# xu-ji/IIC

Measured on AMD Instinct MI355X. Metric: paired-images/sec, STL10 96x96 ClusterNet5g+IID_loss, higher is better.
Workload: dtype bf16; 1 GPU; STL10 96x96 ClusterNet5g IID+ (cluster_sobel.py train step), batch 660 pairs/GPU, 5 sub-heads, k=70, bf16 MFMA convs / fp32 stem+heads+loss, fused HIP Adam; global_batch_pairs=660, input=96x96x1 grey -> sobel 2ch, parallelism=dp1, streams=2, launch=hip-graph replay: 6 linear graph segments, the two views on two streams

## Files before the change

iic_amd/csrc/conv_igemm_bd.hip:

```cpp
#include "common.h"
#include "conv_plan.h"
#include "conv_tile.h"
#include "../../include/iic_hip.h"

template <int OFF>
__device__ __forceinline__ void bd_bload_at(u32x4& d, unsigned voff, const unsigned char* sbase) {
  asm volatile("global_load_dwordx4 %0, %1, %2 offset:%3" : "=v"(d) : "v"(voff), "s"(sbase), "n"(OFF) : "memory");
}
__device__ __forceinline__ void bd_bload(u32x4& d, unsigned voff, const unsigned char* sbase, int ks) {
  switch (ks) {
    case 0: bd_bload_at<0>(d, voff, sbase); break;
    case 1: bd_bload_at<1024>(d, voff, sbase); break;
    case 2: bd_bload_at<2048>(d, voff, sbase); break;
    default: bd_bload_at<3072>(d, voff, sbase); break;
  }
}
template <int N>
__device__ __forceinline__ void bd_bwait(u32x4& d) {
  asm volatile("s_waitcnt vmcnt(%1)" : "+v"(d) : "i"(N) : "memory");
}


#define BD_BM 256
#define BD_BN 128
// ... 326 lines not shown
  if (PROF) t_stamp[4] = __builtin_readcyclecounter();
  TileRed tr;
  if (RED) tile_red_zero(tr);
  if (!(ABL & 32))
    igemm_store_tile<BNT, BM, BD_THREADS, 8, RED, (BM == 256 ? BD_STORE_UB : 4)>(sC, s_pout, out, res_grad, res_act, accumulate,
                                                                 g.Cout, n0, tid, red_y, red_coef, red_y2, &tr);
  if (RED)
    igemm_red_finish<BNT, BD_THREADS, RED>(tr, reinterpret_cast<float*>(smem_raw), red_stats, red_stats2,
                                             g.Cout, n0, tid);
  if (PROF && prof && tid == 0) {
    unsigned long long* q = prof + (long)blockIdx.x * BD_PROF_SLOTS;
    const unsigned long long t_end = __builtin_readcyclecounter();
    q[0] = t_stamp[0]; q[1] = t_stamp[1]; q[2] = t_stamp[2]; q[3] = t_stamp[3]; q[4] = t_stamp[4];
    q[5] = t_end; q[6] = t_bsum; q[7] = (unsigned long long)t_nb;
    q[8] = iic_hw_stamp();
    q[9] = (unsigned long long)tix;
    q[10] = __builtin_amdgcn_s_memrealtime();
  }
}

template <bool GATHER, int ABL, int MS, int RED, int WN = 2, bool PAD = false>
__global__ __launch_bounds__(BD_THREADS, ((MS == 4 || WN == 1) ? 2 : 3)) void conv_igemm_bd_kernel(
    const iic_conv_geom g, const bf16_t* __restrict__ in, const unsigned char* __restrict__ wfrag,
    bf16_t* __restrict__ out, float* __restrict__ stats, const bf16_t* __restrict__ res_grad,
    const bf16_t* __restrict__ res_act, int accumulate, int num_mtiles, int lds_a_bytes,
    const bf16_t* __restrict__ red_y, const float* __restrict__ red_coef,
    const bf16_t* __restrict__ red_y2, float* __restrict__ red_stats, float* __restrict__ red_stats2,
    unsigned long long* __restrict__ prof, const bd_blk B) {
  bd_tile<GATHER, ABL, MS, RED, WN, PAD>(g, in, wfrag, out, stats, res_grad, res_act, accumulate, lds_a_bytes, red_y,
                                    red_coef, red_y2, red_stats, red_stats2, prof, (int)blockIdx.x,
                                    num_mtiles * (g.Cout / (WN * 64)), B);
}

__global__ void weight_prep_frag_kernel(const float* __restrict__ w, bf16_t* __restrict__ o, int Co,
                                        int Ci, int T, int mode) {
  const int Nn = mode ? Ci : Co, Kk = mode ? Co : Ci;
  const int n32 = Nn >> 5, nchunks = Kk >> 6;
  const long total = (long)T * Co * Ci;
  for (long i = (long)blockIdx.x * blockDim.x + threadIdx.x; i < total;
       i += (long)gridDim.x * blockDim.x) {
    const int e = (int)(i & 7), lane = (int)((i >> 3) & 63), ks = (int)((i >> 9) & 3);
    long r = i >> 11;
    const int j = (int)(r % n32);
    r /= n32;
    const int kc = (int)(r % nchunks), t = (int)(r / nchunks);
    const int n = j * 32 + (lane & 31), k = kc * 64 + ks * 16 + (lane >> 5) * 8 + e;
    const int co = mode ? k : n, ci = mode ? n : k;
    o[i] = f32_to_bf16(w[((long)co * Ci + ci) * T + t]);
  }
}

IIC_SWITCH(g_p64_enabled, 1, iic_debug_enable_p64)
IIC_SWITCH(g_p64_red, 0, iic_debug_p64_red)

extern "C" {

#ifdef IIC_DEBUG_HOOKS
static unsigned long long* g_bd_prof = nullptr;
IIC_HOOK void iic_debug_bd_prof(void* buf) { g_bd_prof = (unsigned long long*)buf; }
IIC_HOOK int iic_debug_bd_prof_slots(void) { return BD_PROF_SLOTS; }
#else
static constexpr unsigned long long* g_bd_prof = nullptr;
#endif

static long bd_lds(long npix, int rows, int couts, bool pad, bool keys, int* lds_a = nullptr) {
  const long a = pad ? pt144_bytes(npix) : (npix * 128 + 1023) & ~1023L;
  const long c = (long)rows * (couts + 8) * 2;
  const long la = ((a > c ? a : c) + 15) & ~15L;
  if (lds_a) *lds_a = (int)la;
  return la + 2L * rows * 4 + 4L * BD_BN * 4 + (keys ? (npix + 15) & ~15L : 0);
}
static long bd_lds_rows(const iic_conv_geom* g, int ms, int wn = 2, bool pad = false, int* lds_a = nullptr) {
  const int rows = ms * 32 * (4 / wn);
  const long npix = g->ntaps == 1 ? rows : (rows >= 192 ? g->NP256 : g->NP);
  const bool skip = g->ntaps > 1 && g->sx == 1 && ((g->in_Wp - g->MX) & 1) == 0 && g->in_Wp != g->MX;
  return bd_lds(npix, rows, wn * 64, pad, !pad && skip, lds_a);
}
IIC_SWITCH(g_bd_pitch144, IIC_BD_PITCH144, iic_debug_bd_pitch144)
#ifdef IIC_DEBUG_HOOKS
IIC_HOOK int iic_debug_get_bd_pitch144(void) { return g_bd_pitch144; }
#endif
static bool bd_pad_ok(const iic_conv_geom* g, int ms) {
// ... 180 lines not shown
    case 128: BD_LAUNCH(false, 128); break;
#endif
    default: BD_LAUNCH(false, 0); break;
  }
  return rc ? rc : iic_launch_status();
}

#ifdef IIC_DEBUG_HOOKS
IIC_HOOK void iic_debug_conv_plan(const iic_conv_geom* g, int* out) {
  conv_plan p;
  conv_make_plan(g, &p);
  const int f[12] = {p.kernel, p.ms, p.wn, p.gather, p.pad, p.blk.bw, p.blk.bh, p.mtiles, p.grid, p.lds_a, (int)p.lds,
                     p.red_ok};
  for (int i = 0; i < 12; ++i) out[i] = f[i];
}
IIC_HOOK int iic_debug_bd_pitch144_used(const iic_conv_geom* g) {
  conv_plan p;
  if (!conv_make_plan(g, &p) || !p.pad) return 0;
  return p.kernel == CONV_PW ? 2 : 1;
}
#endif

__global__ __launch_bounds__(256) void weight_prep_multi_kernel(const iic_weight_prep_job* __restrict__ jobs,
                                                                int njobs) {
  int lo = 0, hi = njobs - 1;
  while (lo < hi) {
    const int mid = (lo + hi + 1) >> 1;
    if ((long long)blockIdx.x >= jobs[mid].first_block) lo = mid; else hi = mid - 1;
  }
  const iic_weight_prep_job j = jobs[lo];
  const float* __restrict__ w = j.w;
  bf16_t* __restrict__ o = reinterpret_cast<bf16_t*>(j.out);
  const int Co = j.Cout, Ci = j.Cin, T = j.T, mode = j.mode;
  const long total = (long)T * Co * Ci;
  const long nblk = (total + 2047) >> 11;
  const long b = (long)blockIdx.x - j.first_block;
  if (b >= nblk) return;
  for (long i = b * 256 + threadIdx.x; i < total; i += nblk * 256) {
    if (mode <= 1) {
      const int Nn = mode ? Ci : Co, Kk = mode ? Co : Ci;
      const int n32 = Nn >> 5, nchunks = Kk >> 6;
      const int e = (int)(i & 7), lane = (int)((i >> 3) & 63), ks = (int)((i >> 9) & 3);
      long r = i >> 11;
      const int jj = (int)(r % n32);
      r /= n32;
      const int kc = (int)(r % nchunks), t = (int)(r / nchunks);
      const int n = jj * 32 + (lane & 31), k = kc * 64 + ks * 16 + (lane >> 5) * 8 + e;
      const int co = mode ? k : n, ci = mode ? n : k;
      o[i] = f32_to_bf16(w[((long)co * Ci + ci) * T + t]);
    } else if (mode == 2) {
      const int ci = (int)(i % Ci);
      const long r = i / Ci;
      const int co = (int)(r % Co), t = (int)(r / Co);
      o[i] = f32_to_bf16(w[((long)co * Ci + ci) * T + t]);
    } else {
      const int co = (int)(i % Co);
      const long r = i / Co;
      const int ci = (int)(r % Ci), t = (int)(r / Ci);
      o[i] = f32_to_bf16(w[((long)co * Ci + ci) * T + t]);
    }
  }
}

long iic_weight_prep_multi_blocks(int Cout, int Cin, int T) { return ((long)T * Cout * Cin + 2047) >> 11; }

int iic_weight_prep_multi(const iic_weight_prep_job* jobs_dev, int njobs, long total_blocks, void* stream) {
  if (!jobs_dev || njobs <= 0 || total_blocks <= 0 || total_blocks >= (1L << 31)) return IIC_ERR_ARG;
  hipLaunchKernelGGL(weight_prep_multi_kernel, dim3((unsigned)total_blocks), dim3(256), 0, (hipStream_t)stream,
                     jobs_dev, njobs);
  return iic_launch_status();
}

int iic_weight_prep_frag(const float* w_oihw, void* w_frag, int Cout, int Cin, int T, int bwd,
                         void* stream) {
  if (!w_oihw || !w_frag || Cout <= 0 || Cin <= 0 || T <= 0) return IIC_ERR_ARG;
  const int Nn = bwd ? Cin : Cout, Kk = bwd ? Cout : Cin;
  if (Nn % 32 != 0 || Kk % 64 != 0) return IIC_ERR_UNSUPPORTED;
  const long total = (long)T * Cout * Cin;
  int grid = (int)((total + 255) / 256);
  if (grid > 4096) grid = 4096;
  hipLaunchKernelGGL(weight_prep_frag_kernel, dim3(grid), dim3(256), 0, (hipStream_t)stream,
                     w_oihw, (bf16_t*)w_frag, Cout, Cin, T, bwd ? 1 : 0);
  return iic_launch_status();
}

}
```

iic_amd/csrc/conv_wgrad.hip:

```cpp
#include "common.h"
#include "conv_plan.h"
#include "conv_tile.h"
#include "../../include/iic_hip.h"

#define BM 128
#define TPG 3
#define NTG 3
#define PFX 4

typedef s16x4 __attribute__((address_space(3))) * lds_s16x4_ptr;

typedef uint16_t __attribute__((address_space(3))) * lds_u16_ptr;
template <bool USE_TR>
__device__ __forceinline__ bf16x8 frag_T(uint32_t a0, uint32_t a1, uint32_t tile, int pitch,
                                         const int* rows8, int col) {
  union { bf16x8 v; s16x4 h[2]; uint16_t e[8]; } u;
  if (USE_TR) {
    u.h[0] = __builtin_amdgcn_ds_read_tr16_b64_v4i16((lds_s16x4_ptr)(uintptr_t)a0);
    u.h[1] = __builtin_amdgcn_ds_read_tr16_b64_v4i16((lds_s16x4_ptr)(uintptr_t)a1);
  } else {
#pragma unroll
    for (int j = 0; j < 8; ++j)
      u.e[j] = *(lds_u16_ptr)(uintptr_t)(tile + rows8[j] * pitch + col * 2);
  }
  return u.v;
}

template <bool USE_TR, bool GATHER, int COT>
__global__ __launch_bounds__(GATHER ? 256 : 768) void conv_wgrad_kernel(
    const iic_conv_geom g, const bf16_t* __restrict__ x, const bf16_t* __restrict__ dy,
    float* __restrict__ partials, int nsplit, int num_ktiles, int lds_x_bytes) {
  constexpr int NT = GATHER ? 256 : 768;
  constexpr int CS = COT / 64;
  constexpr int DPITCH = COT == 64 ? 144 : 288;
  constexpr int DPIECES = BM * (COT / 8);
  constexpr int PDN = (DPIECES + NT - 1) / NT;
  constexpr int MYT = GATHER ? 1 : TPG;
  extern __shared__ __attribute__((aligned(16))) unsigned char smem_raw[];
  unsigned char* sX = smem_raw;
  unsigned char* sD = smem_raw + lds_x_bytes;
  int* s_pin = reinterpret_cast<int*>(sD + BM * DPITCH);
  int* s_pout = s_pin + 2 * BM;

  const int tid = threadIdx.x, lane = tid & 63, wave = tid >> 6;
  const int tg = wave >> 2, wm = (wave >> 1) & 1, wn = wave & 1;
  const int l31 = lane & 31, g5 = lane >> 5;
  const int q = lane >> 4, i16 = lane & 15;
  const int ncit = g.Cin >> 6;
  int tile = blockIdx.x, split = blockIdx.y;
  if ((gridDim.y & 7) == 0) {
    const int L = blockIdx.y * gridDim.x + blockIdx.x;
    const int xcd = L & 7, j = L >> 3;
    tile = j % (int)gridDim.x;
    split = xcd + 8 * (j / (int)gridDim.x);
  }
  const int cot = tile / ncit, cit = tile - cot * ncit;
  const int co0 = cot * COT, ci0 = cit * 64;
  const int per = (num_ktiles + nsplit - 1) / nsplit;
  const int kt0 = split * per;
  const int kt1 = min(num_ktiles, kt0 + per);
  const int in_pixels = g.N * g.in_Hp * g.in_Wp;
// ... 56 lines not shown
      }
    }
  };
  auto lstore_x = [&]() {
    const int tl = launder(tid);
#pragma unroll
    for (int u = 0; u < PFX; ++u) {
      const int idx = u * NT + tl;
      if (idx < n8) *reinterpret_cast<u32x4*>(sX + (idx >> 3) * ROWB + (idx & 7) * 16) = PX[u];
    }
  };
  auto load_x_sync_big = [&](int b) {
    const int p_lo = s_pin[b * BM];
    for (int base = 0; base < n8; base += NT * 4) {
      u32x4 v[4];
#pragma unroll
      for (int u = 0; u < 4; ++u) {
        const int idx = base + u * NT + tid;
        v[u] = (u32x4){0u, 0u, 0u, 0u};
        if (idx < n8) {
          const int p = p_lo + (idx >> 3);
          if (p < in_pixels)
            v[u] = *reinterpret_cast<const u32x4*>(x + ((long)p * g.Cin + ci0 + (idx & 7) * 8));
        }
      }
#pragma unroll
      for (int u = 0; u < 4; ++u) {
        const int idx = base + u * NT + tid;
        if (idx < n8) *reinterpret_cast<u32x4*>(sX + (idx >> 3) * ROWB + (idx & 7) * 16) = v[u];
      }
    }
  };

  for (int t0 = (int)blockIdx.z * (GATHER ? 1 : NTG * TPG), pass = 0; pass < 1; ++pass) {
    const int tfirst = t0 + tg * MYT;
    const int tcount = max(0, min(MYT, g.ntaps - tfirst));
    f32x16 acc[MYT][CS];
#pragma unroll
    for (int t = 0; t < MYT; ++t)
#pragma unroll
      for (int c = 0; c < CS; ++c)
#pragma unroll
        for (int r = 0; r < 16; ++r) acc[t][c][r] = 0.f;

    __syncthreads();
    if (kt0 < kt1) {
      rowinfo(kt0, 0);
      __syncthreads();
      gload_d(0);
      if (pf) { gload_x(0); lstore_x(); } else load_x_sync_big(0);
      lstore_d();
      if (kt0 + 1 < kt1) rowinfo(kt0 + 1, 1);
      __syncthreads();
    }
    for (int kt = kt0; kt < kt1; ++kt) {
      const int b = (kt - kt0) & 1;
      const bool more = kt + 1 < kt1;
      if (more) {
        gload_d(b ^ 1);
        if (pf) gload_x(b ^ 1);
      }
      const int p_lo = s_pin[b * BM];
      const int* spin = s_pin + b * BM;
#pragma unroll 2
      for (int ks = 0; ks < BM / 16; ++ks) {
        int rows8[8], rowsA[8];
// ... 72 lines not shown
    for (int u = 0; u < 8; ++u) a[u] = 0.f;
    int sp = 0;
    for (; sp + 8 <= nsplit; sp += 8) {
#pragma unroll
      for (int u = 0; u < 8; ++u) a[u] += partials[(long)(sp + u) * per + i];
    }
    for (; sp < nsplit; ++sp) a[0] += partials[(long)sp * per + i];
    const float s = ((a[0] + a[1]) + (a[2] + a[3])) + ((a[4] + a[5]) + (a[6] + a[7]));
    const int ci = (int)(i % Ci);
    const long r = i / Ci;
    const int co = (int)(r % Co), t = (int)(r / Co);
    const long o = ((long)co * Ci + ci) * T + t;
    dW[o] = accumulate ? dW[o] + s : s;
  }
}

__global__ void probe_tr16_kernel(uint16_t* out) {
  __shared__ __attribute__((aligned(16))) uint16_t lds[64 * 4];
  const int l = threadIdx.x;
  for (int i = l; i < 256; i += 64) lds[i] = (uint16_t)i;
  __syncthreads();
  const s16x4 v = __builtin_amdgcn_ds_read_tr16_b64_v4i16((lds_s16x4_ptr)(&lds[l * 4]));
  for (int j = 0; j < 4; ++j) out[l * 4 + j] = (uint16_t)v[j];
}

extern "C" {

#ifdef IIC_DEBUG_HOOKS
static int g_wgrad_target_wgs = 224;
IIC_HOOK void iic_debug_wgrad_target_wgs(int v) { g_wgrad_target_wgs = v > 0 ? v : 224; }
#else
static constexpr int g_wgrad_target_wgs = 224;
#endif

static int wgrad_reg_kt(const iic_conv_geom* g) { return (int)((igemm_rows_host(g) + BM - 1) / BM); }
static int wgrad_reg_batches(const iic_conv_geom* g) { return g->ntaps == 1 ? 1 : (g->ntaps + NTG * TPG - 1) / (NTG * TPG); }

int iic_conv_wgrad_nsplit(const iic_conv_geom* g) {
  const int kt = wgrad_reg_kt(g);
  const int tiles = (g->Cout / wgrad_cot(g)) * (g->Cin / 64) * wgrad_reg_batches(g);
  int ns = g_wgrad_target_wgs / (tiles > 0 ? tiles : 1);
  if (ns < 1) ns = 1;
  if (ns > kt) ns = kt;
  return ns;
}

static bool wgrad_make_plan(const iic_conv_geom* g, int use_tr, wgrad_plan* p) {
  *p = wgrad_plan{};
  if (!g || g->Cin % 64 != 0 || g->Cout % 64 != 0 || g->ntaps < 1 || g->ntaps > IIC_MAX_TAPS) return false;
  if (igemm_rows_host(g) >= (1L << 31) || (long)g->N * g->in_Hp * g->in_Wp >= (1L << 31)) return false;
  p->use_tr = use_tr != 0;
  p->cot = wgrad_cot(g);
  p->gx = (g->Cout / p->cot) * (g->Cin / 64);
  p->nsplit = iic_conv_wgrad_nsplit(g);
  if (use_tr && iic_wgrad_dma_plan(g, p)) return true;
  p->gather = g->ntaps == 1;
  p->bmk = BM; p->nbuf = 1;
  p->np = p->gather ? BM : g->NP;
  p->lx = (p->np * ROWB + 15) & ~15;
  p->lds = (long)p->lx + BM * (p->cot == 64 ? 144 : 288) + 4 * BM * 4;
  if (p->lds > IIC_LDS_BYTES) {
    *p = wgrad_plan{};
    return false;
  }
  p->kt = wgrad_reg_kt(g);
  p->gz = wgrad_reg_batches(g);
  p->threads = p->gather ? 256 : 768;
  p->kernel = WGRAD_REG;
  return true;
}

int iic_conv_wgrad(const iic_conv_geom* g, const void* x, const void* dy, float* partials,
                   int nsplit, int use_tr, void* stream) {
  if (!g || !x || !dy || !partials || nsplit < 1) return IIC_ERR_ARG;
  wgrad_plan p;
  if (!wgrad_make_plan(g, use_tr, &p)) return IIC_ERR_UNSUPPORTED;
  if (p.kernel != WGRAD_REG) return iic_wgrad_dma_launch(g, p, x, dy, partials, nsplit, stream);
  int rc = IIC_OK;
#define WGRAD_LAUNCH(TR_, GA_, COT_)                                                                           \
  rc = iic_launch_lds<conv_wgrad_kernel<TR_, GA_, COT_>>(dim3(p.gx, nsplit, p.gz), dim3(p.threads), p.lds,     \
                                                         (hipStream_t)stream, *g, (const bf16_t*)x,            \
                                                         (const bf16_t*)dy, partials, nsplit, p.kt, p.lx)
#define WGRAD_LAUNCH2(TR_, GA_)                                                                 \
  do {                                                                                          \
    if (p.cot == 128) WGRAD_LAUNCH(TR_, GA_, 128); else WGRAD_LAUNCH(TR_, GA_, 64);             \
  } while (0)
  if (p.use_tr) { if (p.gather) WGRAD_LAUNCH2(true, true); else WGRAD_LAUNCH2(true, false); }
  else          { if (p.gather) WGRAD_LAUNCH2(false, true); else WGRAD_LAUNCH2(false, false); }
  return rc ? rc : iic_launch_status();
}

#ifdef IIC_DEBUG_HOOKS
IIC_HOOK void iic_debug_wgrad_plan(const iic_conv_geom* g, int use_tr, int* out) {
  wgrad_plan p;
  wgrad_make_plan(g, use_tr, &p);
  const int f[28] = {p.kernel, p.band > 0, p.asm_reads, p.gather, p.cot, p.bmk, p.nbuf, p.ntab, p.txs, p.band,
                     p.bstride, p.mto, p.np, p.plane, p.lx, p.kt, p.gx, p.nsplit, p.gz, p.threads, (int)p.lds,
                     p.blk.bw, p.blk.bh, p.blk.nbx, p.blk.nby, p.blk.PW, p.blk.NPR, p.blk.drow};
  for (int i = 0; i < 28; ++i) out[i] = f[i];
}
#endif

int iic_conv_wgrad_reduce(const float* partials, int nsplit, int T, int Cout, int Cin, float* dW,
                          int accumulate, void* stream) {
  if (!partials || !dW || nsplit < 1) return IIC_ERR_ARG;
  const long per = (long)T * Cout * Cin;
  int grid = (int)((per + 255) / 256);
  if (grid > 4096) grid = 4096;
  hipLaunchKernelGGL(conv_wgrad_reduce_kernel, dim3(grid), dim3(256), 0, (hipStream_t)stream,
                     partials, nsplit, T, Cout, Cin, dW, accumulate);
  return iic_launch_status();
}

int iic_probe_tr16(void* out_u16_64x4, void* stream) {
  hipLaunchKernelGGL(probe_tr16_kernel, dim3(1), dim3(64), 0, (hipStream_t)stream,
                     (uint16_t*)out_u16_64x4);
  return iic_launch_status();
}

}
```

iic_amd/csrc/bn.hip:

```cpp
#include "common.h"
#include "../../include/iic_hip.h"

__device__ __forceinline__ void unpack8(const uint4 v, float* f) {
  f[0] = bf16lo(v.x); f[1] = bf16hi(v.x); f[2] = bf16lo(v.y); f[3] = bf16hi(v.y);
  f[4] = bf16lo(v.z); f[5] = bf16hi(v.z); f[6] = bf16lo(v.w); f[7] = bf16hi(v.w);
}
__device__ __forceinline__ uint4 pack8(const float* f) {
  return make_uint4(pack_bf16x2(f[0], f[1]), pack_bf16x2(f[2], f[3]), pack_bf16x2(f[4], f[5]),
                    pack_bf16x2(f[6], f[7]));
}

template <bool NT>
__device__ __forceinline__ uint4 ld16(const bf16_t* p) {
  if (NT) {
    const u32x4 v = __builtin_nontemporal_load(reinterpret_cast<const u32x4*>(p));
    return make_uint4(v[0], v[1], v[2], v[3]);
  }
  return *reinterpret_cast<const uint4*>(p);
}
__global__ __launch_bounds__(256) void bn_finalize_kernel(
    float* __restrict__ stats, const float* __restrict__ gamma, const float* __restrict__ beta,
    float* __restrict__ running_mean, float* __restrict__ running_var, long long* __restrict__ nbt,
    float* __restrict__ coef, int C, long count, long ucount, float eps, float momentum, int training) {
  const int lane16 = threadIdx.x & 15;
// ... 207 lines not shown
  unpack8(*reinterpret_cast<const uint4*>(y + off), v);
  if (act) {
    float a[8];
    unpack8(*reinterpret_cast<const uint4*>(act + off), a);
#pragma unroll
    for (int i = 0; i < 8; ++i) g[i] = a[i] > 0.f ? g[i] : 0.f;
  } else if (mcoef) {
    ld8(mcoef + c8 * 8, k1);
    ld8(mcoef + C + c8 * 8, k2);
#pragma unroll
    for (int i = 0; i < 8; ++i) g[i] = (v[i] * k1[i] + k2[i]) > 0.f ? g[i] : 0.f;
  }
  ld8(bcoef + c8 * 8, k1);
  ld8(bcoef + C + c8 * 8, k2);
  ld8(bcoef + 2 * C + c8 * 8, k3);
#pragma unroll
  for (int i = 0; i < 8; ++i) o[i] = k1[i] * g[i] + k2[i] * v[i] + k3[i];
  *reinterpret_cast<uint4*>(dy + off) = pack8(o);
  if (y2) {
    unpack8(*reinterpret_cast<const uint4*>(y2 + off), v);
    ld8(bcoef2 + c8 * 8, k1);
    ld8(bcoef2 + C + c8 * 8, k2);
    ld8(bcoef2 + 2 * C + c8 * 8, k3);
#pragma unroll
    for (int i = 0; i < 8; ++i) o[i] = k1[i] * g[i] + k2[i] * v[i] + k3[i];
    *reinterpret_cast<uint4*>(dy2 + off) = pack8(o);
  }
}

struct PxWalk {
  int x, yy;
  long off;
};
__device__ __forceinline__ PxWalk px_start(long q, int H, int W, int P, int C, int c8) {
  const long row = q / W;
  PxWalk w;
  w.x = (int)(q - row * W);
  const long n = row / H;
  w.yy = (int)(row - n * H);
  const int Hp = H + 2 * P, Wp = W + 2 * P;
  w.off = ((n * Hp + w.yy + P) * Wp + P + w.x) * C + c8 * 8;
  return w;
}
__device__ __forceinline__ void px_advance(PxWalk& w, int step, int H, int W, int P, int C) {
  w.x += step;
  w.off += (long)step * C;
  while (w.x >= W) {
    w.x -= W;
    w.off += 2L * P * C;
    if (++w.yy == H) {
      w.yy = 0;
      w.off += 2L * P * (W + 2 * P) * C;
    }
  }
}

template <int MASK, bool HAS2, bool NTL>
__global__ __launch_bounds__(256) void bn_bwd_reduce2_kernel(
    const bf16_t* __restrict__ dout, const bf16_t* __restrict__ act, const bf16_t* __restrict__ y,
    const bf16_t* __restrict__ y2, float* __restrict__ sums, float* __restrict__ sums2,
    const float* __restrict__ mcoef, long npx, long per, int H, int W, int P, int C) {
  __shared__ float s_acc[256 * 8];
  const int c8n = C >> 3;
  const int PL = 256 / c8n;
  const int c8 = threadIdx.x % c8n, pl = threadIdx.x / c8n;
  float sg[8], sgy[8], sgy2[HAS2 ? 8 : 1], msc[MASK == 2 ? 8 : 1], msh[MASK == 2 ? 8 : 1];
#pragma unroll
  for (int i = 0; i < 8; ++i) sg[i] = sgy[i] = 0.f;
  if (HAS2) {
#pragma unroll
    for (int i = 0; i < 8; ++i) sgy2[HAS2 ? i : 0] = 0.f;
  }
  if (MASK == 2) {
#pragma unroll
    for (int i = 0; i < 8; ++i) {
      msc[MASK == 2 ? i : 0] = mcoef[c8 * 8 + i];
      msh[MASK == 2 ? i : 0] = mcoef[C + c8 * 8 + i];
    }
  }
  const long q0 = (long)blockIdx.x * per;
  const long q1 = q0 + per < npx ? q0 + per : npx;
  auto accumulate = [&](const uint4 rg, const uint4 ra, const uint4 ry, const uint4 ry2) {
    float g[8], v[8];
    unpack8(rg, g);
    if (MASK == 1) {
      float a[8];
// ... 307 lines not shown
long iic_stat_bytes(int C) {
  return C > 0 ? (long)IIC_STAT_STRIPES * C * 2 * IIC_STAT_BINS * (long)sizeof(iic_stat_t) : 0;
}

int iic_bn_running_update(int n, const float* const* coef, float* const* running_mean,
                          float* const* running_var, long long* const* num_batches_tracked,
                          const int* C, float momentum, void* stream) {
  if (n <= 0 || !coef || !running_mean || !running_var || !num_batches_tracked || !C) return IIC_ERR_ARG;
  int base = 0;
  while (base < n) {
    BnRunTable t;
    int cnt = 0, maxC = 0;
    while (base + cnt < n && cnt < BNRU_CHUNK) {
      const int j = base + cnt;
      bool dup = false;
      for (int k = 0; k < cnt; ++k) dup = dup || t.rm[k] == running_mean[j];
      if (dup) break;
      if (!coef[j] || !running_mean[j] || !running_var[j] || C[j] <= 0) return IIC_ERR_ARG;
      t.coef[cnt] = coef[j]; t.rm[cnt] = running_mean[j]; t.rv[cnt] = running_var[j];
      t.nbt[cnt] = num_batches_tracked[j]; t.C[cnt] = C[j];
      if (C[j] > maxC) maxC = C[j];
      ++cnt;
    }
    for (int k = cnt; k < BNRU_CHUNK; ++k) { t.coef[k] = nullptr; t.rm[k] = nullptr; t.rv[k] = nullptr; t.nbt[k] = nullptr; t.C[k] = 0; }
    hipLaunchKernelGGL(bn_running_update_kernel, dim3((maxC + 255) / 256, cnt), dim3(256), 0,
                       (hipStream_t)stream, t, momentum);
    base += cnt;
  }
  return iic_launch_status();
}

static int check_c(int C) { return (C % 64 == 0 && 256 % (C / 8) == 0 && C <= 2048) ? 0 : 1; }

int iic_bn_apply(const void* y, const float* coef, const void* res, const void* y2,
                 const float* coef2, void* out, int N, int H, int W, int P, int C, int relu,
                 void* stream) {
  if (!y || !coef || !out || N <= 0 || H <= 0 || W <= 0) return IIC_ERR_ARG;
  if (C % 8 != 0) return IIC_ERR_UNSUPPORTED;
  if ((y2 == nullptr) != (coef2 == nullptr)) return IIC_ERR_ARG;
  dim3 grid(N * H, (W * (C / 8) + 255) / 256);
#define BN_APPLY_LAUNCH(L_)                                                                                 \
  hipLaunchKernelGGL((bn_apply_kernel<L_>), grid, dim3(256), 0, (hipStream_t)stream, (const bf16_t*)y, coef, \
                     (const bf16_t*)res, (const bf16_t*)y2, coef2, (bf16_t*)out, H, W, P, C, relu)
  if (g_bn_nt) BN_APPLY_LAUNCH(true); else BN_APPLY_LAUNCH(false);
  return iic_launch_status();
}

int iic_bn_bwd_reduce(const void* dout, const void* act, const void* y, const void* y2, float* sums,
                      float* sums2, const float* mask_coef, int N, int H, int W, int P, int C,
                      void* stream) {
  if (!dout || !y || !sums || N <= 0 || (act && mask_coef)) return IIC_ERR_ARG;
  if (check_c(C)) return IIC_ERR_UNSUPPORTED;
  if ((y2 == nullptr) != (sums2 == nullptr)) return IIC_ERR_ARG;
  const int mode = act ? 1 : (mask_coef ? 2 : 0);
  if (g_bn_v2) {
    long per;
    int grid2;
    bn_v2_grid((long)N * H * W, C, per, grid2, 1);
#define BN_RED2_LAUNCH_(M_, H2_, L_)                                                            \
  hipLaunchKernelGGL((bn_bwd_reduce2_kernel<M_, H2_, L_>), dim3(grid2), dim3(256), 0,           \
                     (hipStream_t)stream, (const bf16_t*)dout, (const bf16_t*)act,              \
                     (const bf16_t*)y, (const bf16_t*)y2, sums, sums2, mask_coef,               \
                     (long)N * H * W, per, H, W, P, C)
#define BN_RED2_LAUNCH(M_, H2_)                                  \
  do {                                                           \
    if (g_bn_nt) BN_RED2_LAUNCH_(M_, H2_, true);                 \
    else BN_RED2_LAUNCH_(M_, H2_, false);                        \
  } while (0)
    if (y2) {
      if (mode == 1) BN_RED2_LAUNCH(1, true); else if (mode == 2) BN_RED2_LAUNCH(2, true); else BN_RED2_LAUNCH(0, true);
    } else {
      if (mode == 1) BN_RED2_LAUNCH(1, false); else if (mode == 2) BN_RED2_LAUNCH(2, false); else BN_RED2_LAUNCH(0, false);
// ... 72 lines not shown
  int grid2;
  bn_v2_grid((long)N * H * W, C, per, grid2, 1);
#define BN_FRZ_LAUNCH_(M_, H2_, L_)                                                              \
  hipLaunchKernelGGL((bn_bwd_frozen_kernel<M_, H2_, L_>), dim3(grid2), dim3(256), 0,            \
                     (hipStream_t)stream, (const bf16_t*)dout, (const bf16_t*)act,              \
                     (const bf16_t*)y, coef, (bf16_t*)dy, (const bf16_t*)y2, coef2,             \
                     (bf16_t*)dy2, sums, sums2, mask_coef, (long)N * H * W, per, H, W, P, C)
#define BN_FRZ_LAUNCH(M_, H2_)                                   \
  do {                                                           \
    if (g_bn_nt) BN_FRZ_LAUNCH_(M_, H2_, true);                  \
    else BN_FRZ_LAUNCH_(M_, H2_, false);                         \
  } while (0)
  if (y2) {
    if (mode == 1) BN_FRZ_LAUNCH(1, true); else if (mode == 2) BN_FRZ_LAUNCH(2, true); else BN_FRZ_LAUNCH(0, true);
  } else {
    if (mode == 1) BN_FRZ_LAUNCH(1, false); else if (mode == 2) BN_FRZ_LAUNCH(2, false); else BN_FRZ_LAUNCH(0, false);
  }
  return iic_launch_status();
}

int iic_bn_bwd_finalize_frozen(float* sums, const float* coef, float* bcoef, float* dgamma, float* dbeta,
                               int C, void* stream) {
  if (!sums || !coef || C <= 0 || (C & 15)) return IIC_ERR_ARG;
  hipLaunchKernelGGL(bn_bwd_finalize_frozen_kernel, dim3((C + 15) / 16), dim3(256), 0,
                     (hipStream_t)stream, sums, coef, bcoef, dgamma, dbeta, C);
  return iic_launch_status();
}

#ifdef IIC_DEBUG_HOOKS
IIC_HOOK void iic_debug_bn_v2(int on, int blocks) {
  g_bn_v2 = on;
  if (blocks > 0) g_bn_v2_blocks = blocks;
}
#endif

}
```

Baseline: 19570 paired-images/sec.

## Pipeline gather wgrad loads across tiles and vectorize weight-prep stores

Adds a software-pipelined path to the gather variant of the wgrad kernel. Global loads for the next DEPTH tiles are held in registers, and row coordinates are advanced incrementally instead of being recomputed with divisions. The aim is to hide global-load latency behind MFMA work, at the cost of more registers per thread and added complexity. The weight-prep kernels are also rewritten so each thread converts 8 elements and writes one 16-byte store, which cuts per-element index math and scalar stores.

Result: no change. 19690 paired-images/sec, median of 6 (+0.6%).

```diff
diff --git a/iic_amd/csrc/conv_igemm_bd.hip b/iic_amd/csrc/conv_igemm_bd.hip
--- a/iic_amd/csrc/conv_igemm_bd.hip
+++ b/iic_amd/csrc/conv_igemm_bd.hip
@@ -382,22 +382,93 @@
                                     num_mtiles * (g.Cout / (WN * 64)), B);
 }
 
-__global__ void weight_prep_frag_kernel(const float* __restrict__ w, bf16_t* __restrict__ o, int Co,
-                                        int Ci, int T, int mode) {
+__device__ __forceinline__ void weight_prep_store8(bf16_t* __restrict__ o, long i, const float* __restrict__ src,
+                                                   long stride) {
+  float f[8];
+#pragma unroll
+  for (int e = 0; e < 8; ++e) f[e] = src[e * stride];
+  const u32x4 v = {pack_bf16x2(f[0], f[1]), pack_bf16x2(f[2], f[3]), pack_bf16x2(f[4], f[5]), pack_bf16x2(f[6], f[7])};
+  if ((reinterpret_cast<uintptr_t>(o) & 15) == 0) {
+    *reinterpret_cast<u32x4*>(o + i) = v;
+  } else {
+#pragma unroll
+    for (int e = 0; e < 4; ++e) {
+      o[i + 2 * e] = (bf16_t)(v[e] & 0xffffu);
+      o[i + 2 * e + 1] = (bf16_t)(v[e] >> 16);
+    }
+  }
+}
+
+__device__ __forceinline__ void weight_prep_divmod(long a, int d, bool small, long& q, int& r) {
+  if (small) {
+    const unsigned qa = (unsigned)a / (unsigned)d;
+    q = qa;
+    r = (int)((unsigned)a - qa * (unsigned)d);
+  } else {
+    q = a / d;
+    r = (int)(a - q * d);
+  }
+}
+
+__device__ __forceinline__ void weight_prep_frag_block(const float* __restrict__ w, bf16_t* __restrict__ o, int Co,
+                                                       int Ci, int T, int mode, long b, int tid) {
   const int Nn = mode ? Ci : Co, Kk = mode ? Co : Ci;
   const int n32 = Nn >> 5, nchunks = Kk >> 6;
+  const bool small = (long)T * Co * Ci < (1L << 31);
+  long grp, kc;
+  int s, j;
+  weight_prep_divmod(b, T, small, grp, s);
+  weight_prep_divmod(grp, n32, small, kc, j);
+  const int u0 = (32 * s) / T, u1 = (32 * (s + 1)) / T;
+  const int ntask = (u1 - u0) * T * 8;
+  for (int q = tid; q < ntask; q += 256) {
+    const int n8 = q & 7, rest = q >> 3;
+    const int ul = (int)((unsigned)rest / (unsigned)T), t = rest - ul * T;
+    const int u = u0 + ul, noct = u & 3, koct = u >> 2;
+    const int n = j * 32 + noct * 8 + n8, k = (int)kc * 64 + koct * 8;
+    const int co = mode ? k : n, ci = mode ? n : k;
+    const long out = ((((long)t * nchunks + kc) * n32 + j) << 11) + ((koct * 32 + noct * 8 + n8) << 3);
+    weight_prep_store8(o, out, w + ((long)co * Ci + ci) * T + t, mode ? (long)Ci * T : (long)T);
+  }
+}
+
+__device__ __forceinline__ void weight_prep_rows_block(const float* __restrict__ w, bf16_t* __restrict__ o, int Co,
+                                                       int Ci, int T, int mode, long b, int tid) {
   const long total = (long)T * Co * Ci;
-  for (long i = (long)blockIdx.x * blockDim.x + threadIdx.x; i < total;
-       i += (long)gridDim.x * blockDim.x) {
-    const int e = (int)(i & 7), lane = (int)((i >> 3) & 63), ks = (int)((i >> 9) & 3);
-    long r = i >> 11;
-    const int j = (int)(r % n32);
-    r /= n32;
-    const int kc = (int)(r % nchunks), t = (int)(r / nchunks);
-    const int n = j * 32 + (lane & 31), k = kc * 64 + ks * 16 + (lane >> 5) * 8 + e;
-    const int co = mode ? k : n, ci = mode ? n : k;
-    o[i] = f32_to_bf16(w[((long)co * Ci + ci) * T + t]);
-  }
+  const int inner = mode == 2 ? Ci : Co, outer = mode == 2 ? Co : Ci;
+  if ((inner & 7) == 0) {
+    const long i = b * 2048 + tid * 8;
+    if (i >= total) return;
+    const bool small = total < (1L << 31);
+    long r, tb;
+    int in_b, out_b;
+    weight_prep_divmod(b * 2048, inner, small, r, in_b);
+    weight_prep_divmod(r, outer, small, tb, out_b);
+    const unsigned c = (unsigned)in_b + (unsigned)tid * 8u;
+    const unsigned q = c / (unsigned)inner, in_i = c - q * (unsigned)inner;
+    const unsigned c2 = (unsigned)out_b + q;
+    const unsigned q2 = c2 / (unsigned)outer, out_i = c2 - q2 * (unsigned)outer;
+    const long t = tb + q2;
+    const long co = mode == 2 ? out_i : in_i, ci = mode == 2 ? in_i : out_i;
+    weight_prep_store8(o, i, w + (co * Ci + ci) * T + t, mode == 2 ? (long)T : (long)Ci * T);
+  } else {
+#pragma unroll 1
+    for (int u = 0; u < 8; ++u) {
+      const long i = b * 2048 + u * 256 + tid;
+      if (i >= total) return;
+      const int in_i = (int)(i % inner);
+      const long r = i / inner;
+      const long out_i = r % outer, t = r / outer;
+      const long co = mode == 2 ? out_i : in_i, ci = mode == 2 ? in_i : out_i;
+      o[i] = f32_to_bf16(w[(co * Ci + ci) * T + t]);
+    }
+  }
+}
+
+__global__ __launch_bounds__(256) void weight_prep_frag_kernel(const float* __restrict__ w, bf16_t* __restrict__ o,
+                                                               int Co, int Ci, int T, int mode) {
+  const long nblk = ((long)T * Co * Ci) >> 11;
+  for (long b = blockIdx.x; b < nblk; b += gridDim.x) weight_prep_frag_block(w, o, Co, Ci, T, mode, b, (int)threadIdx.x);
 }
 
 IIC_SWITCH(g_p64_enabled, 1, iic_debug_enable_p64)
@@ -644,34 +715,12 @@
   const float* __restrict__ w = j.w;
   bf16_t* __restrict__ o = reinterpret_cast<bf16_t*>(j.out);
   const int Co = j.Cout, Ci = j.Cin, T = j.T, mode = j.mode;
-  const long total = (long)T * Co * Ci;
-  const long nblk = (total + 2047) >> 11;
+  const long nblk = ((long)T * Co * Ci + 2047) >> 11;
   const long b = (long)blockIdx.x - j.first_block;
   if (b >= nblk) return;
-  for (long i = b * 256 + threadIdx.x; i < total; i += nblk * 256) {
-    if (mode <= 1) {
-      const int Nn = mode ? Ci : Co, Kk = mode ? Co : Ci;
-      const int n32 = Nn >> 5, nchunks = Kk >> 6;
-      const int e = (int)(i & 7), lane = (int)((i >> 3) & 63), ks = (int)((i >> 9) & 3);
-      long r = i >> 11;
-      const int jj = (int)(r % n32);
-      r /= n32;
-      const int kc = (int)(r % nchunks), t = (int)(r / nchunks);
-      const int n = jj * 32 + (lane & 31), k = kc * 64 + ks * 16 + (lane >> 5) * 8 + e;
-      const int co = mode ? k : n, ci = mode ? n : k;
-      o[i] = f32_to_bf16(w[((long)co * Ci + ci) * T + t]);
-    } else if (mode == 2) {
-      const int ci = (int)(i % Ci);
-      const long r = i / Ci;
-      const int co = (int)(r % Co), t = (int)(r / Co);
-      o[i] = f32_to_bf16(w[((long)co * Ci + ci) * T + t]);
-    } else {
-      const int co = (int)(i % Co);
-      const long r = i / Co;
-      const int ci = (int)(r % Ci), t = (int)(r / Ci);
-      o[i] = f32_to_bf16(w[((long)co * Ci + ci) * T + t]);
-    }
-  }
+  if (mode <= 1 && (b + 1) * 2048 > (long)T * Co * Ci) return;
+  if (mode <= 1) weight_prep_frag_block(w, o, Co, Ci, T, mode, b, (int)threadIdx.x);
+  else weight_prep_rows_block(w, o, Co, Ci, T, mode, b, (int)threadIdx.x);
 }
 
 long iic_weight_prep_multi_blocks(int Cout, int Cin, int T) { return ((long)T * Cout * Cin + 2047) >> 11; }
@@ -688,9 +737,8 @@
   if (!w_oihw || !w_frag || Cout <= 0 || Cin <= 0 || T <= 0) return IIC_ERR_ARG;
   const int Nn = bwd ? Cin : Cout, Kk = bwd ? Cout : Cin;
   if (Nn % 32 != 0 || Kk % 64 != 0) return IIC_ERR_UNSUPPORTED;
-  const long total = (long)T * Cout * Cin;
-  int grid = (int)((total + 255) / 256);
-  if (grid > 4096) grid = 4096;
+  const long nblk = ((long)T * Cout * Cin) >> 11;
+  const int grid = (int)(nblk < 4096 ? nblk : 4096);
   hipLaunchKernelGGL(weight_prep_frag_kernel, dim3(grid), dim3(256), 0, (hipStream_t)stream,
                      w_oihw, (bf16_t*)w_frag, Cout, Cin, T, bwd ? 1 : 0);
   return iic_launch_status();
diff --git a/iic_amd/csrc/conv_wgrad.hip b/iic_amd/csrc/conv_wgrad.hip
--- a/iic_amd/csrc/conv_wgrad.hip
+++ b/iic_amd/csrc/conv_wgrad.hip
@@ -26,7 +26,35 @@
   return u.v;
 }
 
-template <bool USE_TR, bool GATHER, int COT>
+struct WgRow { int n, y, x; };
+struct WgStep { int d_n, d_y, d_x; };
+__device__ __forceinline__ WgStep wg_step(int rows, int mp, int MX) {
+  WgStep s;
+  s.d_n = rows / mp;
+  const int r = rows - s.d_n * mp;
+  s.d_y = r / MX;
+  s.d_x = r - s.d_y * MX;
+  return s;
+}
+__device__ __forceinline__ WgRow wg_row_init(int m, int mp, int MX) {
+  WgRow r;
+  r.n = m / mp;
+  const int q = m - r.n * mp;
+  r.y = q / MX;
+  r.x = q - r.y * MX;
+  return r;
+}
+__device__ __forceinline__ void wg_row_advance(WgRow& r, const WgStep& s, int MX, int Ym, int Xm) {
+  r.n += s.d_n; r.y += s.d_y; r.x += s.d_x;
+  const bool cx = r.x >= MX;
+  r.x -= cx ? MX : 0; r.y += cx ? 1 : 0;
+  const bool cp = (r.y > Ym) | ((r.y == Ym) & (r.x >= Xm));
+  r.x -= cp ? Xm : 0; r.y -= cp ? Ym : 0; r.n += cp ? 1 : 0;
+  const bool bx = r.x < 0;
+  r.x += bx ? MX : 0; r.y -= bx ? 1 : 0;
+}
+
+template <bool USE_TR, bool GATHER, int COT, int DEPTH = 0>
 __global__ __launch_bounds__(GATHER ? 256 : 768) void conv_wgrad_kernel(
     const iic_conv_geom g, const bf16_t* __restrict__ x, const bf16_t* __restrict__ dy,
     float* __restrict__ partials, int nsplit, int num_ktiles, int lds_x_bytes) {
@@ -149,6 +177,144 @@
     }
   };
 
+  if constexpr (GATHER && DEPTH > 0) {
+    constexpr int DR = COT / 8;
+    constexpr int DPR = DR / 8;
+    constexpr int NR = PFX;
+    static_assert(DR % 8 == 0 && NR * (NT / 8) == BM && PDN == NR * DPR && DPIECES == PDN * NT, "whole rows per thread");
+    static_assert(DEPTH <= 4, "the tile loop below is written out for up to 4 stages");
+    const int tfirst = (int)blockIdx.z;
+    const bool has_tap = tfirst < g.ntaps;
+    f32x16 acc[CS];
+#pragma unroll
+    for (int c = 0; c < CS; ++c)
+#pragma unroll
+      for (int r = 0; r < 16; ++r) acc[c][r] = 0.f;
+
+    if (kt0 < kt1 && has_tap) {
+      const int plane = g.MY * g.MX, mp = g.MP > 0 ? g.MP : plane, MX = g.MX;
+      const int Ym = mp / MX, Xm = mp - Ym * MX;
+      const WgStep st_tile = wg_step(BM, mp, MX), st_row = wg_step(NT / 8, mp, MX);
+      const int cA = g.in_Hp * g.in_Wp, cB = g.sy * g.in_Wp, cD = g.oy * g.in_Wp + g.ox;
+      const int oA = g.out_Hp * g.out_Wp, oB = g.ty * g.out_Wp, oD = g.py * g.out_Wp + g.px;
+      const int xcol = ci0 + (tid & 7) * 8, dcol = co0 + (tid & 7) * 8;
+      WgRow rw[NR];
+      rw[0] = wg_row_init(kt0 * BM + (tid >> 3), mp, MX);
+#pragma unroll
+      for (int u = 1; u < NR; ++u) { rw[u] = rw[u - 1]; wg_row_advance(rw[u], st_row, MX, Ym, Xm); }
+
+      auto opaque = [](long v) { asm("" : "+v"(v)); return v; };
+      constexpr uint32_t ALL = (1u << (2 * NR)) - 1u;
+      u32x4 SX[DEPTH][PFX], SD[DEPTH][PDN];
+      uint32_t vm[DEPTH];
+      auto gload = [&](u32x4 (&sx)[PFX], u32x4 (&sd)[PDN], uint32_t& m, bool live) {
+        m = 0u;
+#pragma unroll
+        for (int u = 0; u < NR; ++u) {
+          const WgRow r = rw[u];
+          const bool inimg = (r.n < g.N) & (r.y < g.MY);
+          const int nn = r.n < g.N ? r.n : g.N - 1, yy = inimg ? r.y : g.MY - 1, xx = inimg ? r.x : MX - 1;
+          const int p = nn * cA + yy * cB + xx * g.sx + cD;
+          const int po = r.n * oA + r.y * oB + r.x * g.tx + oD;
+          const bool okx = live & (p < in_pixels), okd = live & inimg;
+          const long ox = opaque(okx ? (long)p * g.Cin + xcol : 0L);
+          const long od = opaque(okd ? (long)po * g.Cout + dcol : 0L);
+          sx[u] = *reinterpret_cast<const u32x4*>(x + ox);
+#pragma unroll
+          for (int v = 0; v < DPR; ++v)
+            sd[u * DPR + v] = *reinterpret_cast<const u32x4*>(dy + od + v * 64);
+          m |= (okx ? 1u << u : 0u) | (okd ? 1u << (NR + u) : 0u);
+          wg_row_advance(rw[u], st_tile, MX, Ym, Xm);
+        }
+      };
+      auto lstore = [&](const u32x4 (&sx)[PFX], const u32x4 (&sd)[PDN], uint32_t m) {
+        unsigned char* px = sX + (tid >> 3) * ROWB + (tid & 7) * 16;
+        unsigned char* pd = sD + (tid >> 3) * DPITCH + (tid & 7) * 16;
+        const u32x4 zero = {0u, 0u, 0u, 0u};
+        if (__builtin_amdgcn_ballot_w64(m != ALL) == 0) {
+#pragma unroll
+          for (int u = 0; u < NR; ++u) {
+            *reinterpret_cast<u32x4*>(px + u * (NT / 8) * ROWB) = sx[u];
+#pragma unroll
+            for (int v = 0; v < DPR; ++v) *reinterpret_cast<u32x4*>(pd + u * (NT / 8) * DPITCH + v * 128) = sd[u * DPR + v];
+          }
+        } else {
+#pragma unroll
+          for (int u = 0; u < NR; ++u) {
+            *reinterpret_cast<u32x4*>(px + u * (NT / 8) * ROWB) = ((m >> u) & 1u) ? sx[u] : zero;
+#pragma unroll
+            for (int v = 0; v < DPR; ++v)
+              *reinterpret_cast<u32x4*>(pd + u * (NT / 8) * DPITCH + v * 128) = ((m >> (NR + u)) & 1u) ? sd[u * DPR + v] : zero;
+          }
+        }
+      };
+      auto mfma_tile = [&]() {
+#pragma unroll
+        for (int ks = 0; ks < BM / 16; ++ks) {
+          int rows8[8];
+          const int k0 = ks * 16 + trow;
+          const uint32_t b0 = sXo + k0 * ROWB + tcolB, b1 = sXo + (k0 + 4) * ROWB + tcolB;
+          if (!USE_TR) {
+#pragma unroll
+            for (int j = 0; j < 8; ++j) rows8[j] = ks * 16 + 8 * g5 + j;
+          }
+          bf16x8 a[CS];
+#pragma unroll
+          for (int c = 0; c < CS; ++c)
+            a[c] = frag_T<USE_TR>(aBase + ks * 16 * DPITCH + c * 64, aBase + (ks * 16 + 4) * DPITCH + c * 64,
+                                  sDo, DPITCH, rows8, wm * (COT / 2) + c * 32 + l31);
+          const bf16x8 bf = frag_T<USE_TR>(b0, b1, sXo, ROWB, rows8, wn * 32 + l31);
+#pragma unroll
+          for (int c = 0; c < CS; ++c)
+            acc[c] = __builtin_amdgcn_mfma_f32_32x32x16_bf16(a[c], bf, acc[c], 0, 0, 0);
+        }
+      };
+
+#pragma unroll
+      for (int s = 0; s < DEPTH; ++s) gload(SX[s], SD[s], vm[s], kt0 + s < kt1);
+      lstore(SX[0], SD[0], vm[0]);
+      __syncthreads();
+      const int ngroups = (kt1 - kt0 - 1) / DEPTH, rem = kt1 - kt0 - ngroups * DEPTH;
+      int kt = kt0;
+#define WG_GATHER_NEXT(S)                                                   \
+  {                                                                         \
+    __syncthreads();                 \
+    lstore(SX[(S) % DEPTH], SD[(S) % DEPTH], vm[(S) % DEPTH]);              \
+    __syncthreads();                                                        \
+  }
+#define WG_GATHER_TILE(S)                                                   \
+  {                                                                         \
+    gload(SX[S], SD[S], vm[S], kt + DEPTH < kt1);                           \
+    mfma_tile();                                                            \
+    ++kt;                                                                   \
+    WG_GATHER_NEXT(S + 1)                                                   \
+  }
+      for (int grp = 0; grp < ngroups; ++grp) {
+        WG_GATHER_TILE(0)
+        if constexpr (DEPTH > 1) WG_GATHER_TILE(1)
+        if constexpr (DEPTH > 2) WG_GATHER_TILE(2)
+        if constexpr (DEPTH > 3) WG_GATHER_TILE(3)
+      }
+      mfma_tile();
+      if constexpr (DEPTH > 1) if (rem > 1) { WG_GATHER_NEXT(1) mfma_tile(); }
+      if constexpr (DEPTH > 2) if (rem > 2) { WG_GATHER_NEXT(2) mfma_tile(); }
+      if constexpr (DEPTH > 3) if (rem > 3) { WG_GATHER_NEXT(3) mfma_tile(); }
+#undef WG_GATHER_TILE
+#undef WG_GATHER_NEXT
+    }
+    if (has_tap) {
+      float* dst = partials + (((long)split * g.ntaps + tfirst) * g.Cout + co0) * g.Cin + ci0;
+#pragma unroll
+      for (int c = 0; c < CS; ++c)
+#pragma unroll
+        for (int r = 0; r < 16; ++r) {
+          const int row = wm * (COT / 2) + c * 32 + mfma32_row(r, lane);
+          dst[(long)row * g.Cin + wn * 32 + l31] = acc[c][r];
+        }
+    }
+    return;
+  }
+
   for (int t0 = (int)blockIdx.z * (GATHER ? 1 : NTG * TPG), pass = 0; pass < 1; ++pass) {
     const int tfirst = t0 + tg * MYT;
     const int tcount = max(0, min(MYT, g.ntaps - tfirst));
@@ -287,6 +453,8 @@
 #else
 static constexpr int g_wgrad_target_wgs = 224;
 #endif
+
+IIC_SWITCH(g_wgrad_gather_depth, 2, iic_debug_wgrad_gather_depth)
 
 static int wgrad_reg_kt(const iic_conv_geom* g) { return (int)((igemm_rows_host(g) + BM - 1) / BM); }
 static int wgrad_reg_batches(const iic_conv_geom* g) { return g->ntaps == 1 ? 1 : (g->ntaps + NTG * TPG - 1) / (NTG * TPG); }
@@ -332,16 +500,29 @@
   if (!wgrad_make_plan(g, use_tr, &p)) return IIC_ERR_UNSUPPORTED;
   if (p.kernel != WGRAD_REG) return iic_wgrad_dma_launch(g, p, x, dy, partials, nsplit, stream);
   int rc = IIC_OK;
-#define WGRAD_LAUNCH(TR_, GA_, COT_)                                                                           \
-  rc = iic_launch_lds<conv_wgrad_kernel<TR_, GA_, COT_>>(dim3(p.gx, nsplit, p.gz), dim3(p.threads), p.lds,     \
-                                                         (hipStream_t)stream, *g, (const bf16_t*)x,            \
-                                                         (const bf16_t*)dy, partials, nsplit, p.kt, p.lx)
-#define WGRAD_LAUNCH2(TR_, GA_)                                                                 \
-  do {                                                                                          \
-    if (p.cot == 128) WGRAD_LAUNCH(TR_, GA_, 128); else WGRAD_LAUNCH(TR_, GA_, 64);             \
+#define WGRAD_LAUNCH(TR_, GA_, COT_, DP_)                                                                         \
+  rc = iic_launch_lds<conv_wgrad_kernel<TR_, GA_, COT_, DP_>>(dim3(p.gx, nsplit, p.gz), dim3(p.threads), p.lds,   \
+                                                              (hipStream_t)stream, *g, (const bf16_t*)x,          \
+                                                              (const bf16_t*)dy, partials, nsplit, p.kt, p.lx)
+#define WGRAD_LAUNCH2(TR_, GA_, DP_)                                                                      \
+  do {                                                                                                    \
+    if (p.cot == 128) WGRAD_LAUNCH(TR_, GA_, 128, DP_); else WGRAD_LAUNCH(TR_, GA_, 64, DP_);             \
   } while (0)
-  if (p.use_tr) { if (p.gather) WGRAD_LAUNCH2(true, true); else WGRAD_LAUNCH2(true, false); }
-  else          { if (p.gather) WGRAD_LAUNCH2(false, true); else WGRAD_LAUNCH2(false, false); }
+#ifdef IIC_DEBUG_HOOKS
+#define WGRAD_LAUNCH_GATHER(TR_)                                          \
+  do {                                                                    \
+    switch (g_wgrad_gather_depth) {                                       \
+      case 0: WGRAD_LAUNCH2(TR_, true, 0); break;                         \
+      case 3: WGRAD_LAUNCH2(TR_, true, 3); break;                         \
+      case 4: WGRAD_LAUNCH2(TR_, true, 4); break;                         \
+      default: WGRAD_LAUNCH2(TR_, true, 2); break;                        \
+    }                                                                     \
+  } while (0)
+#else
+#define WGRAD_LAUNCH_GATHER(TR_) WGRAD_LAUNCH2(TR_, true, g_wgrad_gather_depth)
+#endif
+  if (p.use_tr) { if (p.gather) WGRAD_LAUNCH_GATHER(true); else WGRAD_LAUNCH2(true, false, 0); }
+  else          { if (p.gather) WGRAD_LAUNCH_GATHER(false); else WGRAD_LAUNCH2(false, false, 0); }
   return rc ? rc : iic_launch_status();
 }
 
```

## Add persistent-range BN apply kernel with unrolled batched loads for large tensors

Applied to the files above, without the earlier changes.

Adds a bn_apply2 kernel in which each block walks a contiguous range of pixels, keeps its per-channel scale and shift in registers, and issues U=4 independent 16-byte loads before computing. This replaces the old one-row-per-block grid. The new path is used only for tensors above a size threshold, or whenever a second BN branch (y2) is fused in. It aims to cut repeated coefficient loads and per-block overhead and to raise memory-level parallelism in a bandwidth-bound elementwise pass. In exchange it adds template variants and a pixel-walk indexing cost.

Measured after the change: 19500 paired-images/sec before, 19610 paired-images/sec after (median of 6 runs). About the same (+0.6%).

```diff
diff --git a/iic_amd/csrc/bn.hip b/iic_amd/csrc/bn.hip
--- a/iic_amd/csrc/bn.hip
+++ b/iic_amd/csrc/bn.hip
@@ -263,7 +263,7 @@
   int x, yy;
   long off;
 };
-__device__ __forceinline__ PxWalk px_start(long q, int H, int W, int P, int C, int c8) {
+__host__ __device__ __forceinline__ PxWalk px_start(long q, int H, int W, int P, int C, int c8) {
   const long row = q / W;
   PxWalk w;
   w.x = (int)(q - row * W);
@@ -283,6 +283,81 @@
       w.yy = 0;
       w.off += 2L * P * (W + 2 * P) * C;
     }
+  }
+}
+
+__host__ __device__ __forceinline__ void bn_apply_range(long b, long per, long npx, long& q0, long& q1) {
+  q0 = b * per;
+  q1 = q0 + per < npx ? q0 + per : npx;
+}
+
+template <int U, bool HAS_RES, bool HAS2, bool NTL>
+__global__ __launch_bounds__(256) void bn_apply2_kernel(
+    const bf16_t* __restrict__ y, const float* __restrict__ coef, const bf16_t* __restrict__ res,
+    const bf16_t* __restrict__ y2, const float* __restrict__ coef2, bf16_t* __restrict__ out,
+    long npx, long per, int H, int W, int P, int C, int relu) {
+  const int c8n = C >> 3;
+  const int PL = 256 / c8n;
+  const int c8 = threadIdx.x % c8n, pl = threadIdx.x / c8n;
+  float sc[8], sh[8], sc2[HAS2 ? 8 : 1], sh2[HAS2 ? 8 : 1];
+#pragma unroll
+  for (int i = 0; i < 8; ++i) {
+    sc[i] = coef[c8 * 8 + i];
+    sh[i] = coef[C + c8 * 8 + i];
+    if (HAS2) {
+      sc2[HAS2 ? i : 0] = coef2[c8 * 8 + i];
+      sh2[HAS2 ? i : 0] = coef2[C + c8 * 8 + i];
+    }
+  }
+  long q0, q1;
+  bn_apply_range(blockIdx.x, per, npx, q0, q1);
+  auto emit = [&](long off, const uint4 ry, const uint4 rr, const uint4 ry2) {
+    float v[8];
+    unpack8(ry, v);
+#pragma unroll
+    for (int i = 0; i < 8; ++i) v[i] = v[i] * sc[i] + sh[i];
+    if (HAS_RES) {
+      float r[8];
+      unpack8(rr, r);
+#pragma unroll
+      for (int i = 0; i < 8; ++i) v[i] += r[i];
+    }
+    if (HAS2) {
+      float r[8];
+      unpack8(ry2, r);
+#pragma unroll
+      for (int i = 0; i < 8; ++i) v[i] += r[i] * sc2[HAS2 ? i : 0] + sh2[HAS2 ? i : 0];
+    }
+    if (relu) {
+#pragma unroll
+      for (int i = 0; i < 8; ++i) v[i] = iic_relu(v[i]);
+    }
+    *reinterpret_cast<uint4*>(out + off) = pack8(v);
+  };
+  long q = q0 + pl;
+  if (q >= q1) return;
+  PxWalk w = px_start(q, H, W, P, C, c8);
+  const uint4 z = make_uint4(0, 0, 0, 0);
+  for (; q + (long)(U - 1) * PL < q1; q += (long)U * PL) {
+    long off[U];
+    uint4 ry[U], rr[U], ry2[U];
+#pragma unroll
+    for (int u = 0; u < U; ++u) {
+      off[u] = w.off;
+      px_advance(w, PL, H, W, P, C);
+    }
+#pragma unroll
+    for (int u = 0; u < U; ++u) {
+      ry[u] = ld16<NTL>(y + off[u]);
+      rr[u] = HAS_RES ? ld16<NTL>(res + off[u]) : z;
+      ry2[u] = HAS2 ? ld16<NTL>(y2 + off[u]) : z;
+    }
+#pragma unroll
+    for (int u = 0; u < U; ++u) emit(off[u], ry[u], rr[u], ry2[u]);
+  }
+  for (; q < q1; q += PL) {
+    emit(w.off, ld16<NTL>(y + w.off), HAS_RES ? ld16<NTL>(res + w.off) : z, HAS2 ? ld16<NTL>(y2 + w.off) : z);
+    px_advance(w, PL, H, W, P, C);
   }
 }
 
@@ -656,12 +731,65 @@
 
 static int check_c(int C) { return (C % 64 == 0 && 256 % (C / 8) == 0 && C <= 2048) ? 0 : 1; }
 
+struct bn_apply_launch {
+  int form, U, unit, grid;
+  long per;
+};
+enum { BN_IN_RES = 1, BN_IN_Y2 = 2 };
+static constexpr int BN_APPLY_BLOCKS = 32768;
+IIC_SWITCH(g_bn_apply_form, 1, iic_debug_bn_apply_form)
+IIC_SWITCH(g_bn_apply_blocks, 0, iic_debug_bn_apply_blocks)
+static bn_apply_launch bn_apply_plan(int N, int H, int W, int C, int inputs) {
+  bn_apply_launch p = {0, 0, 0, 0, 0};
+  if (!g_bn_apply_form || check_c(C)) return p;
+  const long npx = (long)N * H * W;
+  const long min_elems = (inputs & BN_IN_Y2) ? 0 : (inputs & BN_IN_RES) ? (1L << 26) : (1L << 25);
+  if (g_bn_apply_form == 1 && npx * C < min_elems) return p;
+  const int PL = 256 / (C >> 3);
+  p.form = 1;
+  p.U = g_bn_apply_form > 1 ? g_bn_apply_form : 4;
+  p.unit = p.U * PL;
+  const int blocks = g_bn_apply_blocks > 0 ? g_bn_apply_blocks : BN_APPLY_BLOCKS;
+  long per = (npx + blocks - 1) / blocks;
+  per = (per + p.unit - 1) / p.unit * p.unit;
+  p.per = per;
+  p.grid = (int)((npx + per - 1) / per);
+  return p;
+}
+
 int iic_bn_apply(const void* y, const float* coef, const void* res, const void* y2,
                  const float* coef2, void* out, int N, int H, int W, int P, int C, int relu,
                  void* stream) {
   if (!y || !coef || !out || N <= 0 || H <= 0 || W <= 0) return IIC_ERR_ARG;
   if (C % 8 != 0) return IIC_ERR_UNSUPPORTED;
   if ((y2 == nullptr) != (coef2 == nullptr)) return IIC_ERR_ARG;
+  const bn_apply_launch pl = bn_apply_plan(N, H, W, C, (res ? BN_IN_RES : 0) | (y2 ? BN_IN_Y2 : 0));
+  if (pl.form) {
+    const long npx = (long)N * H * W;
+#define BN_APPLY2_LAUNCH_(U_, R_, H2_, L_)                                                                      \
+  hipLaunchKernelGGL((bn_apply2_kernel<U_, R_, H2_, L_>), dim3(pl.grid), dim3(256), 0, (hipStream_t)stream,     \
+                     (const bf16_t*)y, coef, (const bf16_t*)res, (const bf16_t*)y2, coef2, (bf16_t*)out, npx,   \
+                     pl.per, H, W, P, C, relu)
+#define BN_APPLY2_LAUNCH(U_)                                                                                    \
+  do {                                                                                                          \
+    if (g_bn_nt) {                                                                                              \
+      if (res) { if (y2) BN_APPLY2_LAUNCH_(U_, true, true, true); else BN_APPLY2_LAUNCH_(U_, true, false, true); }    \
+      else { if (y2) BN_APPLY2_LAUNCH_(U_, false, true, true); else BN_APPLY2_LAUNCH_(U_, false, false, true); }      \
+    } else {                                                                                                    \
+      if (res) { if (y2) BN_APPLY2_LAUNCH_(U_, true, true, false); else BN_APPLY2_LAUNCH_(U_, true, false, false); }  \
+      else { if (y2) BN_APPLY2_LAUNCH_(U_, false, true, false); else BN_APPLY2_LAUNCH_(U_, false, false, false); }    \
+    }                                                                                                           \
+  } while (0)
+    switch (pl.U) {
+      case 4: BN_APPLY2_LAUNCH(4); break;
+#ifdef IIC_DEBUG_HOOKS
+      case 2: BN_APPLY2_LAUNCH(2); break;
+      case 8: BN_APPLY2_LAUNCH(8); break;
+#endif
+      default: return IIC_ERR_UNSUPPORTED;
+    }
+    return iic_launch_status();
+  }
   dim3 grid(N * H, (W * (C / 8) + 255) / 256);
 #define BN_APPLY_LAUNCH(L_)                                                                                 \
   hipLaunchKernelGGL((bn_apply_kernel<L_>), grid, dim3(256), 0, (hipStream_t)stream, (const bf16_t*)y, coef, \
@@ -800,6 +928,15 @@
   g_bn_v2 = on;
   if (blocks > 0) g_bn_v2_blocks = blocks;
 }
+IIC_HOOK void iic_debug_bn_apply_plan(int N, int H, int W, int C, int inputs, long* out) {
+  const bn_apply_launch p = bn_apply_plan(N, H, W, C, inputs);
+  out[0] = p.form; out[1] = p.U; out[2] = p.unit; out[3] = p.grid; out[4] = p.per;
+}
+IIC_HOOK void iic_debug_bn_apply_block(long b, long per, long npx, int H, int W, int P, int C, long* out) {
+  bn_apply_range(b, per, npx, out[0], out[1]);
+  out[2] = px_start(out[0], H, W, P, C, 0).off;
+  out[3] = px_start(out[1] - 1, H, W, P, C, 0).off;
+}
 #endif
 
 }
```
